# astomodynamics/cddp-cpp

Measured on AMD Instinct MI355X. Metric: trajectories_per_sec, higher is better.
Workload: dtype f64

## Files before the change

### cddp-cpp_amd/csrc/dev_models.hpp

```cpp
#pragma once
#include "dev_linalg.hpp"
#include "dev_trig.hpp"
#include "../../include/cddp_hip.h"

namespace cddp_dev {

template <int NP>
struct DualN {
  double v;
  double d[NP];
  DEV DualN() {}
  DEV DualN(double x) : v(x) {
#pragma unroll
    for (int i = 0; i < NP; ++i) d[i] = 0.0;
  }
};
template <int NP> DEV DualN<NP> operator+(const DualN<NP> &a, const DualN<NP> &b) { DualN<NP> r; r.v = a.v + b.v;
#pragma unroll
  for (int i = 0; i < NP; ++i) r.d[i] = a.d[i] + b.d[i]; return r; }
template <int NP> DEV DualN<NP> operator-(const DualN<NP> &a, const DualN<NP> &b) { DualN<NP> r; r.v = a.v - b.v;
#pragma unroll
  for (int i = 0; i < NP; ++i) r.d[i] = a.d[i] - b.d[i]; return r; }
template <int NP> DEV DualN<NP> operator-(const DualN<NP> &a) { DualN<NP> r; r.v = -a.v;
#pragma unroll
  for (int i = 0; i < NP; ++i) r.d[i] = -a.d[i]; return r; }
template <int NP> DEV DualN<NP> operator*(const DualN<NP> &a, const DualN<NP> &b) { DualN<NP> r; r.v = a.v * b.v;
#pragma unroll
  for (int i = 0; i < NP; ++i) r.d[i] = a.d[i] * b.v + a.v * b.d[i]; return r; }
template <int NP> DEV DualN<NP> operator/(const DualN<NP> &a, const DualN<NP> &b) { DualN<NP> r; r.v = a.v / b.v;
#pragma unroll
  for (int i = 0; i < NP; ++i) r.d[i] = (a.d[i] - r.v * b.d[i]) / b.v; return r; }
template <int NP> DEV DualN<NP> dsin(const DualN<NP> &a) { DualN<NP> r; double s, c; plant_sincos(a.v, &s, &c); r.v = s;
#pragma unroll
  for (int i = 0; i < NP; ++i) r.d[i] = c * a.d[i]; return r; }
template <int NP> DEV DualN<NP> dcos(const DualN<NP> &a) { DualN<NP> r; double s, c; plant_sincos(a.v, &s, &c); r.v = c; double ms = -s;
#pragma unroll
  for (int i = 0; i < NP; ++i) r.d[i] = ms * a.d[i]; return r; }
template <int NP> DEV DualN<NP> dsqrt(const DualN<NP> &a) { DualN<NP> r; r.v = sqrt(a.v); double g = 0.5 / r.v;
#pragma unroll
  for (int i = 0; i < NP; ++i) r.d[i] = g * a.d[i]; return r; }
template <int NP> DEV DualN<NP> dasin(const DualN<NP> &a) { DualN<NP> r; r.v = plant_asin(a.v); double g = 1.0 / sqrt(1.0 - a.v * a.v);
#pragma unroll
  for (int i = 0; i < NP; ++i) r.d[i] = g * a.d[i]; return r; }
template <int NP> DEV DualN<NP> dtan(const DualN<NP> &a) { DualN<NP> r; r.v = plant_tan(a.v); double g = 1.0 + r.v * r.v;
#pragma unroll
  for (int i = 0; i < NP; ++i) r.d[i] = g * a.d[i]; return r; }
DEV double dasin(double a) { return plant_asin(a); }
DEV double dtan(double a) { return plant_tan(a); }
DEV double dsin(double a) { return plant_sin(a); }
DEV double dcos(double a) { return plant_cos(a); }
DEV double dsqrt(double a) { return sqrt(a); }
DEV double dval(double a) { return a; }
template <int NP> DEV double dval(const DualN<NP> &a) { return a.v; }
DEV double lift_sin(double, double s, double) { return s; }
DEV double lift_cos(double, double, double c) { return c; }
template <int NP> DEV DualN<NP> lift_sin(const DualN<NP> &a, double s, double c) { DualN<NP> r; r.v = s;
#pragma unroll
  for (int i = 0; i < NP; ++i) r.d[i] = c * a.d[i]; return r; }
template <int NP> DEV DualN<NP> lift_cos(const DualN<NP> &a, double s, double c) { DualN<NP> r; r.v = c; const double ms = -s;
#pragma unroll
  for (int i = 0; i < NP; ++i) r.d[i] = ms * a.d[i]; return r; }
template <int N, class S> DEV void trig_n(const S *a, S *sn, S *cs) {
  double av[N], sv[N], cv[N];
#pragma unroll
  for (int i = 0; i < N; ++i) av[i] = dval(a[i]);
  sincos_n<N>(av, sv, cv);
#pragma unroll
  for (int i = 0; i < N; ++i) { sn[i] = lift_sin(a[i], sv[i], cv[i]); cs[i] = lift_cos(a[i], sv[i], cv[i]); }
}

template <int NP>
struct Dual2N {
  double v, d[NP], h[NP * NP];
  DEV Dual2N() {}
  DEV Dual2N(double x) : v(x) {
    for (int i = 0; i < NP; ++i) d[i] = 0.0;
    for (int i = 0; i < NP * NP; ++i) h[i] = 0.0;
  }
};
template <int NP> DEV Dual2N<NP> d2_unary(const Dual2N<NP> &a, double val, double p1, double p2) {
  Dual2N<NP> r; r.v = val;
  for (int i = 0; i < NP; ++i) { r.d[i] = p1 * a.d[i]; for (int j = 0; j < NP; ++j) r.h[i * NP + j] = p2 * a.d[i] * a.d[j] + p1 * a.h[i * NP + j]; }
  return r;
}
template <int NP> DEV Dual2N<NP> operator+(const Dual2N<NP> &a, const Dual2N<NP> &b) { Dual2N<NP> r; r.v = a.v + b.v;
  for (int i = 0; i < NP; ++i) r.d[i] = a.d[i] + b.d[i];
  for (int i = 0; i < NP * NP; ++i) r.h[i] = a.h[i] + b.h[i]; return r; }
template <int NP> DEV Dual2N<NP> operator-(const Dual2N<NP> &a, const Dual2N<NP> &b) { Dual2N<NP> r; r.v = a.v - b.v;
// ... 45 lines not shown
      D xs[NX], us[NU], xd[NX];
      for (int v = 0; v < NP; ++v) {
        D z(v < NX ? x[v] : u[v - NX]);
        const int blk = v / BS, off = v - blk * BS;
        if (blk == I) z.d[off] = 1.0;
        else if (blk == J) z.d[BS + off] = 1.0;
        if (v < NX) xs[v] = z; else us[v - NX] = z;
      }
      F::template eval<D>(p, xs, us, xd);
      for (int pass = 0; pass < (I == J ? 1 : 2); ++pass) {
        const int RB = pass == 0 ? I : J, CB = pass == 0 ? J : I;
        for (int ra = 0; ra < BS; ++ra) {
          const int va = RB * BS + ra;
          if (va >= NP) break;
          const int sa = (RB == I) ? ra : BS + ra;
          for (int cb = 0; cb < BS; ++cb) {
            const int vb = CB * BS + cb;
            if (vb >= NP) break;
            const int sb = (CB == I) ? cb : BS + cb;
            double *dst;
            if (va < NX && vb < NX) dst = Qxx + va * NX + vb;
            else if (va >= NX && vb >= NX) dst = Quu + (va - NX) * NU + (vb - NX);
            else if (va >= NX && vb < NX) dst = Qux + (va - NX) * NX + vb;
            else continue;
            double acc = *dst;
            for (int i = 0; i < NX; ++i) acc = acc + w[i] * (dt * (xd[i].h[sa * NS + sb] / div));
            *dst = acc;
          }
        }
      }
    }
  }
}

template <class M, class = void> struct HessBlocked { static constexpr bool value = false; };
template <class M> struct HessBlocked<M, decltype((void)sizeof(typename M::HessDyn))> { static constexpr bool value = true; };

template <class F, int NX, int NU>
DEV void ad_jacobian(const double *p, const double *x, const double *u, double *Fx, double *Fu) {
  typedef DualN<NX + NU> D;
  D xs[NX], us[NU], xd[NX];
#pragma unroll
  for (int i = 0; i < NX; ++i) { xs[i] = D(x[i]); xs[i].d[i] = 1.0; }
#pragma unroll
  for (int j = 0; j < NU; ++j) { us[j] = D(u[j]); us[j].d[NX + j] = 1.0; }
  F::template eval<D>(p, xs, us, xd);
#pragma unroll
  for (int i = 0; i < NX; ++i) {
#pragma unroll
    for (int j = 0; j < NX; ++j) Fx[i * NX + j] = xd[i].d[j];
#pragma unroll
    for (int j = 0; j < NU; ++j) Fu[i * NU + j] = xd[i].d[NX + j];
  }
}

struct PendulumModel {
  static constexpr int ID = CDDP_HIP_MODEL_PENDULUM, NX = 2, NU = 1;
  static constexpr bool kDiscrete = false;
  DEV static void f(const double *p, const double *x, const double *u, double *xd) {
    const double length = p[0], mass = p[1], damping = p[2], gravity = p[3];
    const double inertia = mass * length * length;
    xd[0] = x[1];
    xd[1] = (u[0] - damping * x[1] + mass * gravity * length * dsin(x[0])) / inertia;
  }
  DEV static void jac(const double *p, const double *x, const double *u, double *Fx, double *Fu) {
    const double length = p[0], mass = p[1], damping = p[2], gravity = p[3];
    Fx[0] = 0.0; Fx[1] = 1.0;
    Fx[2] = (gravity / length) * dcos(x[0]);
    Fx[3] = -damping / (mass * length * length);
    Fu[0] = 0.0; Fu[1] = 1.0 / (mass * length * length);
  }
  static constexpr bool kHasHess = true;
  DEV static void hess(const double *p, const double *x, const double *, double *Fxx, double *Fuu, double *Fux) {
    for (int i = 0; i < NX * NX * NX; ++i) Fxx[i] = 0.0;
    for (int i = 0; i < NX * NU * NU; ++i) Fuu[i] = 0.0;
    for (int i = 0; i < NX * NU * NX; ++i) Fux[i] = 0.0;
    Fxx[1 * NX * NX + 0] = -(p[3] / p[0]) * dsin(x[0]);
  }
};

struct CartPoleModel {
  static constexpr int ID = CDDP_HIP_MODEL_CARTPOLE, NX = 4, NU = 1;
  static constexpr bool kDiscrete = false;
  DEV static void f(const double *p, const double *x, const double *u, double *xd) {
    const double mc = p[0], mp = p[1], l = p[2], g = p[3];
    const double theta_dot = x[3], force = u[0];
    double s, c; plant_sincos(x[1], &s, &c);
    const double total_mass = mc + mp;
    const double den = mc + mp * s * s;
    xd[0] = x[2];
    xd[1] = theta_dot;
    xd[2] = (force + mp * s * (l * theta_dot * theta_dot + g * c)) / den;
    xd[3] = (-force * c - mp * l * theta_dot * theta_dot * c * s - total_mass * g * s) / (l * den);
  }
  DEV static void jac(const double *p, const double *x, const double *u, double *Fx, double *Fu) {
#ifdef CDDP_TRIG_SHARED
    {
      typedef DualN<5> D;
      D xs[4], us[1], xd[4];
#pragma unroll
      for (int i = 0; i < 4; ++i) { xs[i] = D(x[i]); xs[i].d[i] = 1.0; }
      us[0] = D(u[0]); us[0].d[4] = 1.0;
      f_ad<D>(p, xs, us, xd);
#pragma unroll
      for (int i = 0; i < 4; ++i) {
#pragma unroll
        for (int j = 0; j < 4; ++j) Fx[i * 4 + j] = xd[i].d[j];
        Fu[i] = xd[i].d[4];
      }
      return;
    }
#endif
    const double mc = p[0], mp = p[1], l = p[2], g = p[3], b = p[4];
    const double w = x[3], F = u[0];
    double s, c; plant_sincos(x[1], &s, &c);
    const double M = mc + mp;
    const double den = mc + mp * s * s;
    const double dden = 2.0 * mp * s * c;
    const double inner = l * w * w + g * c;
    const double num3 = F + mp * s * inner;
    const double dnum3 = mp * c * inner - mp * s * g * s;
    const double num4 = -F * c - mp * l * w * w * c * s - M * g * s - b * w;
    const double dnum4 = F * s - mp * l * w * w * (c * c - s * s) - M * g * c;
    const double den2 = den * den;
#pragma unroll
    for (int i = 0; i < 16; ++i) Fx[i] = 0.0;
    Fx[0 * 4 + 2] = 1.0;
    Fx[1 * 4 + 3] = 1.0;
    Fx[2 * 4 + 1] = (dnum3 * den - num3 * dden) / den2;
    Fx[2 * 4 + 3] = (mp * s * (2.0 * l * w)) / den;
    Fx[3 * 4 + 1] = (dnum4 * den - num4 * dden) / (l * den2);
    Fx[3 * 4 + 3] = (-2.0 * mp * l * w * c * s - b) / (l * den);
    Fu[0] = 0.0; Fu[1] = 0.0;
    Fu[2] = 1.0 / den;
    Fu[3] = -c / (l * den);
  }
  template <class S>
  DEV static void f_ad(const double *p, const S *x, const S *u, S *xd) {
    const double mc = p[0], mp = p[1], l = p[2], g = p[3], b = p[4];
    const S theta = x[1], x_dot = x[2], theta_dot = x[3], force = u[0];
    const S sin_theta = dsin(theta), cos_theta = dcos(theta);
    const double total_mass = mc + mp;
    const S den = S(mc) + S(mp) * sin_theta * sin_theta;
    xd[0] = x_dot;
    xd[1] = theta_dot;
    xd[2] = (force + S(mp) * sin_theta * (S(l) * theta_dot * theta_dot + S(g) * cos_theta)) / den;
    xd[3] = (-force * cos_theta - S(mp) * S(l) * theta_dot * theta_dot * cos_theta * sin_theta - S(total_mass) * S(g) * sin_theta - S(b) * theta_dot) / (S(l) * den);
  }
  static constexpr bool kHasHess = true;
  DEV static void hess(const double *p, const double *x, const double *u, double *Fxx, double *Fuu, double *Fux) {
    typedef Dual2N<5> D;
    D xs[4], us[1], xd[4];
    for (int i = 0; i < 4; ++i) { xs[i] = D(x[i]); xs[i].d[i] = 1.0; }
    us[0] = D(u[0]); us[0].d[4] = 1.0;
    f_ad<D>(p, xs, us, xd);
    for (int i = 0; i < 4; ++i) {
      for (int a = 0; a < 4; ++a) for (int b = 0; b < 4; ++b) Fxx[i * 16 + a * 4 + b] = xd[i].h[a * 5 + b];
      Fuu[i] = xd[i].h[4 * 5 + 4];
      for (int b = 0; b < 4; ++b) Fux[i * 4 + b] = xd[i].h[4 * 5 + b];
    }
  }
};

struct UnicycleModel {
  static constexpr int ID = CDDP_HIP_MODEL_UNICYCLE, NX = 3, NU = 2;
  static constexpr bool kDiscrete = false;
  DEV static void f(const double *, const double *x, const double *u, double *xd) {
    double s, c; plant_sincos(x[2], &s, &c);
    xd[0] = u[0] * c; xd[1] = u[0] * s; xd[2] = u[1];
  }
  DEV static void jac(const double *, const double *x, const double *u, double *Fx, double *Fu) {
    double s, c; plant_sincos(x[2], &s, &c);
#pragma unroll
    for (int i = 0; i < 9; ++i) Fx[i] = 0.0;
    Fx[0 * 3 + 2] = -u[0] * s;
    Fx[1 * 3 + 2] = u[0] * c;
    Fu[0] = c; Fu[1] = 0.0; Fu[2] = s; Fu[3] = 0.0; Fu[4] = 0.0; Fu[5] = 1.0;
  }
  static constexpr bool kHasHess = true;
  DEV static void hess(const double *, const double *x, const double *u, double *Fxx, double *Fuu, double *Fux) {
    double s, c; plant_sincos(x[2], &s, &c);
    for (int i = 0; i < NX * NX * NX; ++i) Fxx[i] = 0.0;
    for (int i = 0; i < NX * NU * NU; ++i) Fuu[i] = 0.0;
    for (int i = 0; i < NX * NU * NX; ++i) Fux[i] = 0.0;
    Fxx[0 * 9 + 2 * 3 + 2] = -u[0] * c;
    Fxx[1 * 9 + 2 * 3 + 2] = -u[0] * s;
    Fux[0 * 6 + 0 * 3 + 2] = -s;
    Fux[1 * 6 + 0 * 3 + 2] = c;
  }
};

template <int NX_, int NU_>
struct LTIModel {
  static constexpr int ID = CDDP_HIP_MODEL_LTI, NX = NX_, NU = NU_;
  static constexpr bool kDiscrete = true;
  static constexpr bool kHasHess = true;
  DEV static void hess(const double *, const double *, const double *, double *Fxx, double *Fuu, double *Fux) {
    for (int i = 0; i < NX * NX * NX; ++i) Fxx[i] = 0.0;
    for (int i = 0; i < NX * NU * NU; ++i) Fuu[i] = 0.0;
    for (int i = 0; i < NX * NU * NX; ++i) Fux[i] = 0.0;
  }
  DEV static void step(const double *p, const double *x, const double *u, double *xn) {
#pragma unroll
    for (int i = 0; i < NX; ++i) {
      double s = 0.0, t = 0.0;
#pragma unroll
      for (int j = 0; j < NX; ++j) s += p[i * NX + j] * x[j];
#pragma unroll
      for (int j = 0; j < NU; ++j) t += p[NX * NX + i * NU + j] * u[j];
      xn[i] = s + t;
    }
  }
  DEV static void f(const double *, const double *, const double *, double *) {}
  DEV static void jac(const double *p, const double *, const double *, double *Fx, double *Fu) {
    const double dt = p[NX * NX + NX * NU];
#pragma unroll
    for (int i = 0; i < NX; ++i)
#pragma unroll
      for (int j = 0; j < NX; ++j) Fx[i * NX + j] = (p[i * NX + j] - (i == j ? 1.0 : 0.0)) / dt;
#pragma unroll
    for (int i = 0; i < NX * NU; ++i) Fu[i] = p[NX * NX + i] / dt;
  }
};

struct BicycleDyn {
  template <class S>
  DEV static void eval(const double *p, const S *x, const S *u, S *xd) {
    const S theta = x[2], v = x[3];
    xd[0] = v * dcos(theta);
    xd[1] = v * dsin(theta);
    xd[2] = (v / S(p[0])) * dtan(u[1]);
    xd[3] = u[0];
  }
};
struct BicycleModel {
  static constexpr int ID = CDDP_HIP_MODEL_BICYCLE, NX = 4, NU = 2;
  static constexpr bool kDiscrete = false;
  static constexpr bool kHasHess = true;
  DEV static void f(const double *p, const double *x, const double *u, double *xd) { BicycleDyn::eval<double>(p, x, u, xd); }
  DEV static void jac(const double *p, const double *x, const double *u, double *Fx, double *Fu) {
    double s, c; plant_sincos(x[2], &s, &c);
    const double v = x[3], L = p[0], cd = plant_cos(u[1]);
#pragma unroll
    for (int i = 0; i < NX * NX; ++i) Fx[i] = 0.0;
#pragma unroll
    for (int i = 0; i < NX * NU; ++i) Fu[i] = 0.0;
    Fx[0 * NX + 2] = -v * s; Fx[0 * NX + 3] = c;
    Fx[1 * NX + 2] = v * c;  Fx[1 * NX + 3] = s;
    Fx[2 * NX + 3] = plant_tan(u[1]) / L;
    Fu[3 * NU + 0] = 1.0;
    Fu[2 * NU + 1] = v / (L * (cd * cd));
// ... 834 lines not shown
      for (int i = 0; i < NX; ++i) xn[i] = x[i] + dt * k1[i];
      return;
    }
    double xt[NX], k2[NX];
    if (integrator == CDDP_HIP_HEUN) {
#pragma unroll
      for (int i = 0; i < NX; ++i) xt[i] = x[i] + dt * k1[i];
      Model::f(p, xt, u, k2);
#pragma unroll
      for (int i = 0; i < NX; ++i) xn[i] = x[i] + (0.5 * dt) * (k1[i] + k2[i]);
      return;
    }
    double k3[NX];
    if (integrator == CDDP_HIP_RK3) {
#pragma unroll
      for (int i = 0; i < NX; ++i) xt[i] = x[i] + (0.5 * dt) * k1[i];
      Model::f(p, xt, u, k2);
#pragma unroll
      for (int i = 0; i < NX; ++i) xt[i] = (x[i] - dt * k1[i]) + (2 * dt) * k2[i];
      Model::f(p, xt, u, k3);
#pragma unroll
      for (int i = 0; i < NX; ++i) xn[i] = x[i] + (dt / 6) * ((k1[i] + 4.0 * k2[i]) + k3[i]);
      return;
    }
    double k4[NX];
#pragma unroll
    for (int i = 0; i < NX; ++i) xt[i] = x[i] + (0.5 * dt) * k1[i];
    Model::f(p, xt, u, k2);
#pragma unroll
    for (int i = 0; i < NX; ++i) xt[i] = x[i] + (0.5 * dt) * k2[i];
    Model::f(p, xt, u, k3);
#pragma unroll
    for (int i = 0; i < NX; ++i) xt[i] = x[i] + dt * k3[i];
    Model::f(p, xt, u, k4);
#pragma unroll
    for (int i = 0; i < NX; ++i) xn[i] = x[i] + (dt / 6) * (((k1[i] + 2.0 * k2[i]) + 2.0 * k3[i]) + k4[i]);
  }
  DEV static void step(const DynCtx &c, const double *x, const double *u, double *xn) {
    constexpr int NX = Model::NX;
    const double *p = c.mp;
    double k1[NX];
    Model::f(p, x, u, k1);
    if (c.integrator == CDDP_HIP_EULER) {
#pragma unroll
      for (int i = 0; i < NX; ++i) xn[i] = x[i] + c.dt * k1[i];
      return;
    }
    double xt[NX], k2[NX];
    if (c.integrator == CDDP_HIP_HEUN) {
#pragma unroll
      for (int i = 0; i < NX; ++i) xt[i] = x[i] + c.dt * k1[i];
      Model::f(p, xt, u, k2);
#pragma unroll
      for (int i = 0; i < NX; ++i) xn[i] = x[i] + c.hdt * (k1[i] + k2[i]);
      return;
    }
    double k3[NX];
    if (c.integrator == CDDP_HIP_RK3) {
#pragma unroll
      for (int i = 0; i < NX; ++i) xt[i] = x[i] + c.hdt * k1[i];
      Model::f(p, xt, u, k2);
#pragma unroll
      for (int i = 0; i < NX; ++i) xt[i] = (x[i] - c.dt * k1[i]) + c.dt2 * k2[i];
      Model::f(p, xt, u, k3);
#pragma unroll
      for (int i = 0; i < NX; ++i) xn[i] = x[i] + c.dt6 * ((k1[i] + 4.0 * k2[i]) + k3[i]);
      return;
    }
    double k4[NX];
#pragma unroll
    for (int i = 0; i < NX; ++i) xt[i] = x[i] + c.hdt * k1[i];
    Model::f(p, xt, u, k2);
#pragma unroll
    for (int i = 0; i < NX; ++i) xt[i] = x[i] + c.hdt * k2[i];
    Model::f(p, xt, u, k3);
#pragma unroll
    for (int i = 0; i < NX; ++i) xt[i] = x[i] + c.dt * k3[i];
    Model::f(p, xt, u, k4);
#pragma unroll
    for (int i = 0; i < NX; ++i) xn[i] = x[i] + c.dt6 * (((k1[i] + 2.0 * k2[i]) + 2.0 * k3[i]) + k4[i]);
  }
};

}
```

### cddp-cpp_amd/csrc/dev_trig.hpp

```cpp
#pragma once
#include <cmath>

#ifndef DEV
#define DEV inline
#define CDDP_TRIG_HOST 1
#endif

namespace cddp_dev {

constexpr double kTrigFastLimit = 1.0e9;

struct SinCosPair { double s, c; };

DEV SinCosPair sincos_fast(double x) {
  const double TWO_OVER_PI = 0x1.45f306dc9c883p-1;
  const double P1 = 0x1.921fb54442d18p+0, P2 = 0x1.1a62633145c07p-54, P3 = -0x1.f1976b7ed8fbcp-110;
  const double dn = __builtin_rint(x * TWO_OVER_PI);
  const double r0 = __builtin_fma(-dn, P1, x);
  const double p = dn * P2;
  const double pe = __builtin_fma(dn, P2, -p);
  const double r = r0 - p;
  const double bb = r - r0;
  const double e1 = (r0 - (r - bb)) + (-p - bb);
  const double y = __builtin_fma(-dn, P3, e1 - pe);
  const double z = r * r, w = z * z;
  const double S1 = -1.66666666666666324348e-01, S2 = 8.33333333332248946124e-03, S3 = -1.98412698298579493134e-04,
               S4 = 2.75573137070700676789e-06, S5 = -2.50507602534068634195e-08, S6 = 1.58969099521155010221e-10;
  const double rs = S2 + z * (S3 + z * S4) + z * w * (S5 + z * S6);
  const double v = z * r;
  const double ks = r - ((z * (0.5 * y - v * rs) - y) - v * S1);
  const double C1 = 4.16666666666666019037e-02, C2 = -1.38888888888741095749e-03, C3 = 2.48015872894767294178e-05,
               C4 = -2.75573143513906633035e-07, C5 = 2.08757232129817482790e-09, C6 = -1.13596475577881948265e-11;
  const double rc = z * (C1 + z * (C2 + z * C3)) + (w * w) * (C4 + z * (C5 + z * C6));
  const double hz = 0.5 * z;
  const double w1 = 1.0 - hz;
  const double kc = w1 + (((1.0 - w1) - hz) + (z * rc - r * y));
  const int n = (int)dn;
  const bool swap = (n & 1) != 0;
  double s = swap ? kc : ks, c = swap ? ks : kc;
  if (n & 2) s = -s;
  if ((n + 1) & 2) c = -c;
  SinCosPair o; o.s = s; o.c = c;
  return o;
}

#ifndef CDDP_TRIG_HOST
__device__ __attribute__((noinline)) inline void sincos_libm(double a, double *s, double *c) { sincos(a, s, c); }
#endif

template <int N>
DEV void sincos_n(const double *a, double *s, double *c) {
  bool slow = false;
#pragma unroll
  for (int i = 0; i < N; ++i) {
    const SinCosPair r = sincos_fast(a[i]);
    s[i] = r.s; c[i] = r.c;
    slow = slow || !(__builtin_fabs(a[i]) < kTrigFastLimit);
  }
#ifdef CDDP_TRIG_HOST
  if (slow)
    for (int i = 0; i < N; ++i)
      if (!(__builtin_fabs(a[i]) < kTrigFastLimit)) { s[i] = std::sin(a[i]); c[i] = std::cos(a[i]); }
#else
  if (__builtin_expect(__builtin_amdgcn_ballot_w64(slow) != 0ull, 0)) {
#pragma unroll
    for (int i = 0; i < N; ++i) {
      double ts, tc;
      sincos_libm(a[i], &ts, &tc);
      const bool out = !(__builtin_fabs(a[i]) < kTrigFastLimit);
      s[i] = out ? ts : s[i];
      c[i] = out ? tc : c[i];
    }
  }
#endif
}

DEV void sincos_1(double a, double *s, double *c) { sincos_n<1>(&a, s, c); }

DEV double bits_to_double(unsigned long long u) { double d; __builtin_memcpy(&d, &u, 8); return d; }
DEV unsigned long long double_to_bits(double d) { unsigned long long u; __builtin_memcpy(&u, &d, 8); return u; }

DEV bool log_fast_ok(double x) { return x >= 0x1p-1022 && x <= 0x1.fffffffffffffp+1023; }
DEV double log_fast_k(double x, int k0) {
  const double ln2_hi = 6.93147180369123816490e-01, ln2_lo = 1.90821492927058770002e-10;
  const double Lg1 = 6.666666666666735130e-01, Lg2 = 3.999999999940941908e-01, Lg3 = 2.857142874366239149e-01,
               Lg4 = 2.222219843214978396e-01, Lg5 = 1.818357216161805012e-01, Lg6 = 1.531383769920937332e-01,
               Lg7 = 1.479819860511658591e-01;
  unsigned long long u = double_to_bits(x);
  unsigned hx = (unsigned)(u >> 32);
  hx += 0x3ff00000u - 0x3fe6a09eu;
  const int k = (int)(hx >> 20) - 0x3ff + k0;
  hx = (hx & 0x000fffffu) + 0x3fe6a09eu;
  u = ((unsigned long long)hx << 32) | (u & 0xffffffffull);
  const double f = bits_to_double(u) - 1.0;
  const double hfsq = 0.5 * f * f;
  const double s = f / (2.0 + f);
  const double z = s * s, w = z * z;
  const double t1 = w * (Lg2 + w * (Lg4 + w * Lg6));
  const double t2 = z * (Lg1 + w * (Lg3 + w * (Lg5 + w * Lg7)));
  const double R = t2 + t1;
  const double dk = (double)k;
  return s * (hfsq + R) + dk * ln2_lo - hfsq + f + dk * ln2_hi;
}
DEV double log_fast(double x) { return log_fast_k(x, 0); }

DEV bool exp_fast_ok(double x) { return __builtin_fabs(x) <= 700.0; }
DEV double exp_fast(double x) {
  const double invln2 = 1.44269504088896338700e+00, ln2hi = 6.93147180369123816490e-01, ln2lo = 1.90821492927058770002e-10;
  const double P1 = 1.66666666666666019037e-01, P2 = -2.77777777770155933842e-03, P3 = 6.61375632143793436117e-05,
               P4 = -1.65339022054652515390e-06, P5 = 4.13813679705723846039e-08;
  const double dk = __builtin_rint(invln2 * x);
  const double hi = x - dk * ln2hi;
  const double lo = dk * ln2lo;
  const double r = hi - lo;
  const double xx = r * r;
  const double c = r - xx * (P1 + xx * (P2 + xx * (P3 + xx * (P4 + xx * P5))));
  const double y = 1.0 + (r * c / (2.0 - c) - lo + hi);
  const int k = (int)dk;
  return y * bits_to_double((unsigned long long)(0x3ff + k) << 52);
}

DEV bool asin_fast_ok(double x) { return __builtin_fabs(x) < 0.5; }
DEV double asin_fast(double x) {
  const double pS0 = 1.66666666666666657415e-01, pS1 = -3.25565818622400915405e-01, pS2 = 2.01212532134862925881e-01,
               pS3 = -4.00555345006794114027e-02, pS4 = 7.91534994289814532176e-04, pS5 = 3.47933107596021167570e-05,
               qS1 = -2.40339491173441421878e+00, qS2 = 2.02094576023350569471e+00, qS3 = -6.88283971605453293030e-01,
               qS4 = 7.70381505559019352791e-02;
  if (__builtin_fabs(x) < 0x1p-26) return x;
// ... 75 lines not shown
```

### cddp-cpp_amd/csrc/kernels_lean.hpp

```cpp
#pragma once
#include "kernels.hpp"

namespace cddp_dev {

#define GI(t, E, e) (((((size_t)(t)) * (size_t)d.NB + (size_t)(b >> 6)) * (E) + (e)) * 64 + (size_t)(b & 63))

template <class Model, class Cons>
struct CstLayout {
  static constexpr int NX = Model::NX, NU = Model::NU;
  static constexpr int CX = 0, CU = CX + NX, WQYU = CU + NU, QYUSIR = WQYU + NU * NU, IPR = QYUSIR + NU, ICOMP = IPR + 1;
  static constexpr int WQYX = ICOMP + 1, QYXSIR = WQYX + NU * NX, WXQYX = QYXSIR + NX;
  static constexpr int SIZE = Cons::HAS_X ? (WXQYX + NX * NX) : WQYX;
};

template <class Model, class Cons, bool WITH_DERIVS>
DEV void condense_eval(const ProblemDev *__restrict__ P, const double *__restrict__ xrt, const int t, const double *x, const double *u,
                       const double *y, const double *s, const double *g, const double mu, double *A, double *Bq, double *c,
                       double *ys_out = nullptr) {
  constexpr int NX = Model::NX, NU = Model::NU, M = Cons::M;
  typedef Objective<NX, NU> Obj;
  typedef CstLayout<Model, Cons> L;
  const double s_floor = dmax(mu * 1e-3, kEpsSlack);
  double Qyx[M * NX], Qyu[M * NU];
  if constexpr (WITH_DERIVS) {
// ... 521 lines not shown
#pragma unroll
    for (int j = 0; j < NX; ++j) s += vb[(size_t)(i * NX + j) * kLS] * dx[j];
    const double lam = (lop[(size_t)i * kLS] + a_pr * vxp[(size_t)i * kLS]) + s;
    finite = finite && dfinite(lam);
    lamp[(size_t)i * kLS] = lam;
  }
  if (!finite || ((d.fail_costate_mask >> only) & 1)) d.t_success[ti] = 2;
}

template <class Model>
__global__ __launch_bounds__(64) void k_costate(DevBuf d, int a0, int na, int phase_req, int force, int first_only) {
  constexpr int NX = Model::NX;
  const int b = blockIdx.x * 64 + threadIdx.x;
  const int t = blockIdx.y;
  if (b >= d.B) return;
  if (!force && d.phase[b] != phase_req) return;
  const int cur = d.cur[b];
  constexpr int NT = NX * (NX + 1) / 2;
  double xo[NX], lo[NX], vx[NX], vt[NT];
  ld<NX>(d.X + (size_t)cur * d.planeX + GI(t, NX, 0), kLS, xo);
  ld<NX>(d.Lam + (size_t)cur * d.planeX + GI(t, NX, 0), kLS, lo);
  ld<NX>(d.Vx + GI(t, NX, 0), kLS, vx);
  costate_load_triangle<NX>(d.Vxx + GI(t, NX * NX, 0), vt);
  int a_lo = a0, a_hi = a0 + na;
  if (first_only != 0) {
    const int only = first_only == 2 ? d.cand[b] : first_surviving_trial(d, a0, na, b);
    if (only < 0) return;
    a_lo = only; a_hi = only + 1;
  }
  for (int a = a_lo; a < a_hi; ++a) {
    const size_t ti = (size_t)a * d.Bp + b;
    if (!d.t_success[ti]) continue;
    const int slot = trial_slot(cur, a);
    const double a_pr = d.t_apr[ti];
    double xn[NX], lam[NX];
    ld<NX>(d.X + (size_t)slot * d.planeX + GI(t, NX, 0), kLS, xn);
    const bool finite = costate_row_eval<NX>(lo, vx, vt, xo, xn, a_pr, lam);
    if (!finite || ((d.fail_costate_mask >> a) & 1)) d.t_success[ti] = 2;
    else st<NX>(d.Lam + (size_t)slot * d.planeX + GI(t, NX, 0), kLS, lam);
  }
}

template <int NX>
DEV void costate_shadow_item(const DevBuf &d, const int b, const int t) {
  if (b >= d.B) return;
  if (d.cs_stampv[b] != d.cs_want) return;
  const int cur = d.cs_old[b], slot = d.cs_new[b];
  const double a_pr = d.cs_apr[b];
  double xo[NX], lo[NX], vx[NX], xn[NX], lam[NX], vt[NX * (NX + 1) / 2];
  ld<NX>(d.X + (size_t)cur * d.planeX + GI(t, NX, 0), kLS, xo);
  ld<NX>(d.Lam + (size_t)cur * d.planeX + GI(t, NX, 0), kLS, lo);
  ld<NX>(d.Vx_prev + GI(t, NX, 0), kLS, vx);
  costate_load_triangle<NX>(d.Vxx_prev + GI(t, NX * NX, 0), vt);
  ld<NX>(d.X + (size_t)slot * d.planeX + GI(t, NX, 0), kLS, xn);
  const bool finite = costate_row_eval<NX>(lo, vx, vt, xo, xn, a_pr, lam);
  if (!finite || (d.cs_fail_stamp != 0 && d.cs_fail_stamp == (d.cs_want | 1))) *d.cs_bad = 1;
  else st<NX>(d.Lam + (size_t)slot * d.planeX + GI(t, NX, 0), kLS, lam);
}

template <class Model>
__global__ __launch_bounds__(64) void k_costate_flush(DevBuf d) {
  costate_shadow_item<Model::NX>(d, blockIdx.x * 64 + threadIdx.x, blockIdx.y);
}

template <int NX>
__global__ __launch_bounds__(64) void k_value_merge(DevBuf d) {
  const int b = blockIdx.x * 64 + threadIdx.x, t = blockIdx.y;
  if (b >= d.B || d.cs_vbuf[b] == d.cs_vsel) return;
  double vx[NX], vxx[NX * NX];
  ld<NX>(d.Vx2 + GI(t, NX, 0), kLS, vx);
  ld<NX * NX>(d.Vxx2 + GI(t, NX * NX, 0), kLS, vxx);
  st<NX>(d.Vx + GI(t, NX, 0), kLS, vx);
  st<NX * NX>(d.Vxx + GI(t, NX * NX, 0), kLS, vxx);
}
#ifdef CDDP_K4_TIMING
__device__ unsigned long long g_k4_times[16384 * 4];
#define K4_TIME_BEGIN const unsigned long long k4_t0 = wall_clock64();
#define K4_TIME_END(role, steps) do { if (lane == 0) { const size_t k4_i = ((size_t)blockIdx.y * gridDim.x + blockIdx.x) * 4 + (role) * 2; \
    g_k4_times[k4_i] = wall_clock64() - k4_t0; g_k4_times[k4_i + 1] = (unsigned long long)(steps); } } while (0)
#else
#define K4_TIME_BEGIN
#define K4_TIME_END(role, steps)
#endif
template <class Model, class Cons, bool TERM = false, int NC = 1>
__global__ __launch_bounds__(64 * (1 + NC)) void k_forward_ipddp_pc(DevBuf d, const ProblemDev *__restrict__ Pk, const double *__restrict__ xrt,
                                                                    int a0, int phase_req, int force) {
  constexpr int NX = Model::NX, NU = Model::NU, M = Cons::M;
  typedef Objective<NX, NU> Obj;
  static_assert(M > 0, "two-role rollout is for path-constrained problems");
  constexpr int RW = 2 * NX + NU;
  constexpr int kRing = RW <= 10 ? 8 : (RW <= 20 ? 4 : 2);
  __shared__ double s_ring[kRing * RW * 64];
  static_assert(NC == 1 || NC == 2, "one or two consumer waves");
  __shared__ int s_prod;
  __shared__ int s_consv[2];
  [[maybe_unused]] __shared__ int s_abort;
  [[maybe_unused]] __shared__ int s_done1;
  constexpr int kL2 = NC > 1 ? 64 : 1;
  [[maybe_unused]] __shared__ int s_pfail[kL2], s_palive[kL2];
  [[maybe_unused]] __shared__ double s_pmax[4 * kL2];
  [[maybe_unused]] __shared__ double s_prun[kL2];
  __shared__ int s_pstat[64];
  __shared__ double s_pcost[64];
  __shared__ double s_xN[TERM ? NX * 64 : 1];
  __shared__ double s_obj[Obj::kStage];
  const int lane = threadIdx.x & 63;
  K4_TIME_BEGIN
  const int wave = __builtin_amdgcn_readfirstlane((int)threadIdx.x) >> 6;
  const bool producer = wave == 0;
  [[maybe_unused]] const int ci = NC > 1 ? wave - 1 : 0;
  int *const s_cons = &s_consv[0];
  const int b = blockIdx.x * 64 + lane;
  const int a = a0 + blockIdx.y;
  const ProblemDev *__restrict__ P = Pk;
  const cddp_hip_options &o = P->opt;
  const int N = d.N;
  const bool active = (b < d.B) && (force || d.phase[b] == phase_req);
  if (__builtin_amdgcn_ballot_w64(active) == 0ull) return;
  if (producer) { s_pstat[lane] = N + 2; if (lane == 0) { s_prod = 0; s_consv[0] = 0; s_consv[1] = 0; if constexpr (NC > 1) { s_abort = 0x7fffffff; s_done1 = 0; } } }
  Obj::stage(P, s_obj, (int)threadIdx.x, 64 * (1 + NC));
  __syncthreads();
  const int bb = (b < d.B) ? b : 0;
  const int cur = (b < d.B) ? d.cur[b] : 0;
  const int slot = trial_slot(cur, a);
  const double *Xc = d.X + (size_t)cur * d.planeX;
  const double alpha = P->alphas[a];
  const double a_pr = dmin(alpha, d.apr_max[bb]);
  auto wait_ge = [&](int *ctr, int need) -> int {
    int v;
    while ((v = __hip_atomic_load(ctr, __ATOMIC_RELAXED, __HIP_MEMORY_SCOPE_WORKGROUP)) < need) __builtin_amdgcn_s_sleep(1);
    asm volatile("" ::: "memory");
    return v;
  };
  const int kAbort = 2 * N + kRing;

  if (producer) {
    double *Xn = d.X + (size_t)slot * d.planeX;
    double *Un = d.U + (size_t)slot * d.planeU;
    const double *Uc = d.U + (size_t)cur * d.planeU;
    bool alive = active;
    double x[NX];
    ld<NX>(Xc + GI(0, NX, 0), kLS, x);
    st<NX>(Xn + GI(0, NX, 0), kLS, x);
    struct StepIn { double xo[NX], uo[NU], kk[NU], KK[NU * NX]; };
    auto load_step = [&](int tt, StepIn &r) {
      ld<NX>(Xc + GI(tt, NX, 0), kLS, r.xo);
      ld<NU>(Uc + GI(tt, NU, 0), kLS, r.uo);
      ld<NU>(d.k + GI(tt, NU, 0), kLS, r.kk);
      ld<NU * NX>(d.K + GI(tt, NU * NX, 0), kLS, r.KK);
    };
    DynCtx dc;
    dc.load(P->integrator, P->dt, P->mp);
    [[maybe_unused]] typename Obj::Ctx oc_p;
    [[maybe_unused]] double run_cost_p = 0.0;
    if constexpr (NC > 1) Obj::load_staged(P, oc_p, s_obj);
    auto prime = [&]() {
      double z[NX];
#pragma unroll
      for (int i = 0; i < NX; ++i) z[i] = 0.0;
      st<NU>(Un + GI(0, NU, 0), kLS, z);
      st<NX>(Xn + GI(1, NX, 0), kLS, z);
    };
    constexpr bool kPing = sizeof(StepIn) <= 40 * sizeof(double);
    constexpr bool kEarly = !kPing && sizeof(StepIn) <= 96 * sizeof(double);
    constexpr bool kChunkP = !kPing && !kEarly;
    struct PChunk { double K[NX], uo, kk; };
    auto load_pchunk = [&](int tt, const int i, PChunk &c) {
      ld<NX>(d.K + GI(tt, NU * NX, i * NX), kLS, c.K);
      c.uo = Uc[GI(tt, NU, i)]; c.kk = d.k[GI(tt, NU, i)];
    };
    PChunk pk0, pk1;
    double xo_c[NX];
    auto step = [&](const int t, StepIn &cs, StepIn &nxt) {
      if constexpr (kPing) {
        const int tn = t + 1 < N ? t + 1 : N - 1;
        load_step(tn, nxt);
      }
      PIPELINE_FENCE();
      double dx[NX], u[NU], xn[NX];
      bool finite = true;
      if constexpr (kChunkP) {
#pragma unroll
        for (int i = 0; i < NX; ++i) dx[i] = x[i] - xo_c[i];
#pragma unroll
        for (int i = 0; i < NU; ++i) {
          if (i + 1 < NU) { if ((i & 1) == 0) load_pchunk(t, i + 1, pk1); else load_pchunk(t, i + 1, pk0); }
          __builtin_amdgcn_sched_barrier(0);
          const PChunk &c = (i & 1) == 0 ? pk0 : pk1;
          double s1 = 0.0;
#pragma unroll
          for (int j = 0; j < NX; ++j) s1 += c.K[j] * dx[j];
          u[i] = (c.uo + a_pr * c.kk) + s1;
          finite = finite && dfinite(u[i]);
          __builtin_amdgcn_sched_barrier(0);
        }
      } else {
#pragma unroll
      for (int i = 0; i < NX; ++i) dx[i] = x[i] - cs.xo[i];
#pragma unroll
      for (int i = 0; i < NU; ++i) {
        double s1 = 0.0;
#pragma unroll
        for (int j = 0; j < NX; ++j) s1 += cs.KK[i * NX + j] * dx[j];
        u[i] = (cs.uo[i] + a_pr * cs.kk[i]) + s1;
        finite = finite && dfinite(u[i]);
      }
      }
      if (t >= kRing && (t % (kRing / 2)) == 0) {
        if (wait_ge(s_cons, t - kRing / 2) >= kAbort) alive = false;
        if constexpr (NC > 1) { if (wait_ge(&s_consv[1], t - kRing / 2) >= kAbort) alive = false; }
      }
      {
        double *rs = s_ring + (size_t)(t % kRing) * RW * 64 + lane;
#pragma unroll
        for (int i = 0; i < NX; ++i) { rs[i * 64] = x[i]; rs[(NX + i) * 64] = dx[i]; }
#pragma unroll
        for (int i = 0; i < NU; ++i) rs[(2 * NX + i) * 64] = u[i];
        if (alive && !finite) { s_pstat[lane] = t; alive = false; }
        RING_FENCE();
        __hip_atomic_store(&s_prod, t + 1, __ATOMIC_RELAXED, __HIP_MEMORY_SCOPE_WORKGROUP);
      }
      if constexpr (NC > 1) run_cost_p += Obj::running_cost(oc_p, xrt, t, x, u);
      if constexpr (kEarly) {
        load_step(t + 1 < N ? t + 1 : t, cs);
        PIPELINE_FENCE();
      }
      if constexpr (kChunkP) {
        const int tn = t + 1 < N ? t + 1 : t;
        ld<NX>(Xc + GI(tn, NX, 0), kLS, xo_c);
        load_pchunk(tn, 0, pk0);
        PIPELINE_FENCE();
      }
      Stepper<Model>::step(dc, x, u, xn);
#pragma unroll
      for (int i = 0; i < NX; ++i) finite = finite && dfinite(xn[i]);
      if (alive && !finite) { s_pstat[lane] = t; alive = false; }
      st<NU>(Un + GI(t, NU, 0), kLS, u);
      st<NX>(Xn + GI(t + 1, NX, 0), kLS, xn);
      if (alive) {
#pragma unroll
        for (int i = 0; i < NX; ++i) x[i] = xn[i];
      }
    };
    StepIn ra;
    int t = 0;
    if constexpr (kPing) {
      StepIn R[2];
#pragma unroll
      for (int j = 0; j < 1; ++j) load_step(j < N ? j : N - 1, R[j]);
      prime();
      for (; t + 1 < N; t += 2) {
#pragma unroll
        for (int j = 0; j <= 1; ++j) step(t + j, R[j], R[(j + 1) % 2]);
        if (__builtin_amdgcn_ballot_w64(alive) == 0ull) { t = N; break; }
      }
#pragma unroll
      for (int j = 0; j <= 1; ++j) if (t + j < N) step(t + j, R[j], R[(j + 1) % 2]);
    } else {
      if constexpr (kChunkP) { ld<NX>(Xc + GI(0, NX, 0), kLS, xo_c); load_pchunk(0, 0, pk0); } else load_step(0, ra);
      prime();
      for (; t < N; ++t) {
        step(t, ra, ra);
        if (__builtin_amdgcn_ballot_w64(alive) == 0ull) break;
      }
    }
    if (alive) s_pcost[lane] = Obj::terminal_cost(P, x);
    if constexpr (NC > 1) s_prun[lane] = run_cost_p;
    if constexpr (TERM) {
#pragma unroll
      for (int i = 0; i < NX; ++i) s_xN[i * 64 + lane] = x[i];
    }
    asm volatile("s_waitcnt lgkmcnt(0)" ::: "memory");
    __hip_atomic_store(&s_prod, N + kRing + 1, __ATOMIC_RELAXED, __HIP_MEMORY_SCOPE_WORKGROUP);
    K4_TIME_END(0, t);
    return;
  }

  const double *Sc = d.S + (size_t)cur * d.planeM;
  const double *Yc = d.Y + (size_t)cur * d.planeM;
  double *Sn = d.S + (size_t)slot * d.planeM;
  double *Yn = d.Y + (size_t)slot * d.planeM;
  double *Gn = d.G + (size_t)slot * d.planeM;
  const double mu = d.mu[bb];
  const double tau = dmax(o.barrier_min_fraction_to_boundary, 1.0 - mu);
  const double a_du = dmin(alpha, d.adu_max[bb]);
  const size_t ti = (size_t)a * d.Bp + bb;
  bool alive = active;
  int seen_prod = 0;
  int fail_t = N;
  if (alive && ci == 0) {
    atomicAdd(d.launched, 1ull);
    d.t_apr[ti] = a_pr; d.t_adu[ti] = a_du;
    d.t_success[ti] = 0;
    d.t_cost[ti] = d.cost[b]; d.t_merit[ti] = d.phi[b]; d.t_theta[ti] = d.theta[b];
    d.t_inf_pr[ti] = 0.0; d.t_inf_comp[ti] = 0.0;
  }
  double ev_total0 = 0.0, ev_max = 0.0, ev_icomp = 0.0, ys_lo = INFINITY, ys_hi = -INFINITY, run_cost = 0.0;
  const bool l2norm = o.ipddp_theta_norm_l2 != 0;
  struct StepIn { double xo[Cons::HAS_X ? NX : 1], uo[Cons::NEEDS_U ? NU : 1], s[M], y[M], ksv[M], ky[M], KK[NU * NX], ys[M]; };
  auto load_step = [&](int tt, StepIn &r) {
    if constexpr (Cons::HAS_X) ld<NX>(Xc + GI(tt, NX, 0), kLS, r.xo);
    if constexpr (Cons::NEEDS_U) ld<NU>(d.U + (size_t)cur * d.planeU + GI(tt, NU, 0), kLS, r.uo);
    ld<M>(Sc + GI(tt, M, 0), kLS, r.s);
    ld<M>(Yc + GI(tt, M, 0), kLS, r.y);
    ld<M>(d.ks + GI(tt, M, 0), kLS, r.ksv);
    ld<M>(d.ky + GI(tt, M, 0), kLS, r.ky);
    ld<NU * NX>(d.K + GI(tt, NU * NX, 0), kLS, r.KK);
    ld<M>(d.ys + GI(tt, M, 0), kLS, r.ys);
  };
  typename Cons::Ctx cc;
  Cons::load(P, cc);
  typename Obj::Ctx oc;
  Obj::load_staged(P, oc, s_obj);
  auto prime = [&]() {
    double z[M];
#pragma unroll
    for (int i = 0; i < M; ++i) z[i] = 0.0;
    const int tp = (NC > 1 && ci < N) ? ci : 0;
    st<M>(Sn + GI(tp, M, 0), kLS, z);
    st<M>(Yn + GI(tp, M, 0), kLS, z);
    st<M>(Gn + GI(tp, M, 0), kLS, z);
    double *ev = d.ev + GI((size_t)a * N + tp, 2 * Cons::NSEG, 0);
#pragma unroll
    for (int c = 0; c < Cons::NSEG; ++c) { if (c > 0 || NC > 1) ev[(size_t)(Cons::NSEG + c) * kLS] = 0.0; ev[(size_t)c * kLS] = 0.0; }
  };
  constexpr bool kPing = sizeof(StepIn) <= 40 * sizeof(double);
  constexpr bool kEarly = !kPing && sizeof(StepIn) <= 96 * sizeof(double);
  constexpr bool kChunk = !kPing && !kEarly && UDiag<Cons>::value && M == 2 * NU;
  struct Chunk { double K[NX], s[2], y[2], ksv[2], ky[2], ys[2]; };
  auto load_chunk = [&](int tt, const int i, Chunk &c) {
    ld<NX>(d.K + GI(tt, NU * NX, i * NX), kLS, c.K);
#pragma unroll
    for (int h = 0; h < 2; ++h) {
      const int r = i + h * NU;
      c.s[h] = Sc[GI(tt, M, r)]; c.y[h] = Yc[GI(tt, M, r)];
      c.ksv[h] = d.ks[GI(tt, M, r)]; c.ky[h] = d.ky[GI(tt, M, r)]; c.ys[h] = d.ys[GI(tt, M, r)];
    }
  };
  Chunk ck0, ck1;
  auto step = [&](const int t, StepIn &cs, StepIn &nxt) {
    if constexpr (kPing) {
      const int tn = t + NC < N ? t + NC : N - 1;
      load_step(tn, nxt);
    } else if constexpr (!kEarly && !kChunk) load_step(t, cs);
    PIPELINE_FENCE();
    if (seen_prod < t + 1) seen_prod = __builtin_amdgcn_readfirstlane(wait_ge(&s_prod, t + 1));
    double rx[NX], dx[NX], u[NU];
// ... 276 lines not shown
```

Measured before the change: 106,800.

## Specialize forward rollout on integrator and defer trig range fallback to wave-level redo

In the ping-pong forward rollout, the integrator choice is hoisted out of the time loop by dispatching to a template instantiated per integrator. Model dynamics for cartpole and unicycle gain a trig policy that uses the fast sincos and only records whether any argument was out of range. When any lane reports that, a noinline checked step recomputes the result. Load and store addresses become incrementing pointers instead of per-step index arithmetic. This aims to cut per-step branching, the inline libm fallback and address math, at the cost of more template instantiations, code size and register pressure.

```diff
diff --git a/cddp-cpp_amd/csrc/dev_models.hpp b/cddp-cpp_amd/csrc/dev_models.hpp
--- a/cddp-cpp_amd/csrc/dev_models.hpp
+++ b/cddp-cpp_amd/csrc/dev_models.hpp
@@ -1,9 +1,25 @@
 #pragma once
+#include <type_traits>
 #include "dev_linalg.hpp"
 #include "dev_trig.hpp"
 #include "../../include/cddp_hip.h"
 
 namespace cddp_dev {
+
+struct TrigChecked {
+  DEV void sincos(double a, double *s, double *c) const { plant_sincos(a, s, c); }
+};
+struct TrigFlagged {
+  bool *out_of_range;
+  DEV void sincos(double a, double *s, double *c) const { const SinCosPair r = sincos_fast_flag(a, *out_of_range); *s = r.s; *c = r.c; }
+};
+#ifdef CDDP_TRIG_SHARED
+constexpr bool kTrigFlaggable = true;
+#else
+constexpr bool kTrigFlaggable = false;
+#endif
+template <class Model, class = void> struct HasTrigPolicy { static constexpr bool value = false; };
+template <class Model> struct HasTrigPolicy<Model, typename std::enable_if<Model::kTrigPolicy>::type> { static constexpr bool value = kTrigFlaggable; };
 
 template <int NP>
 struct DualN {
@@ -215,10 +231,12 @@
 struct CartPoleModel {
   static constexpr int ID = CDDP_HIP_MODEL_CARTPOLE, NX = 4, NU = 1;
   static constexpr bool kDiscrete = false;
-  DEV static void f(const double *p, const double *x, const double *u, double *xd) {
+  static constexpr bool kTrigPolicy = true;
+  template <class Trig = TrigChecked>
+  DEV static void f(const double *p, const double *x, const double *u, double *xd, const Trig tg = Trig()) {
     const double mc = p[0], mp = p[1], l = p[2], g = p[3];
     const double theta_dot = x[3], force = u[0];
-    double s, c; plant_sincos(x[1], &s, &c);
+    double s, c; tg.sincos(x[1], &s, &c);
     const double total_mass = mc + mp;
     const double den = mc + mp * s * s;
     xd[0] = x[2];
@@ -298,8 +316,10 @@
 struct UnicycleModel {
   static constexpr int ID = CDDP_HIP_MODEL_UNICYCLE, NX = 3, NU = 2;
   static constexpr bool kDiscrete = false;
-  DEV static void f(const double *, const double *x, const double *u, double *xd) {
-    double s, c; plant_sincos(x[2], &s, &c);
+  static constexpr bool kTrigPolicy = true;
+  template <class Trig = TrigChecked>
+  DEV static void f(const double *, const double *x, const double *u, double *xd, const Trig tg = Trig()) {
+    double s, c; tg.sincos(x[2], &s, &c);
     xd[0] = u[0] * c; xd[1] = u[0] * s; xd[2] = u[1];
   }
   DEV static void jac(const double *, const double *x, const double *u, double *Fx, double *Fu) {
@@ -1300,4 +1320,56 @@
   }
 };
 
+template <class Model, bool FLAGGED, class Trig>
+DEV void roll_f(const double *p, const double *x, const double *u, double *xd, const Trig tg) {
+  if constexpr (FLAGGED) Model::f(p, x, u, xd, tg);
+  else Model::f(p, x, u, xd);
 }
+template <class Model, int INTEG, bool FLAGGED = HasTrigPolicy<Model>::value>
+DEV void roll_step(const DynCtx &c, const double *x, const double *u, double *xn, bool *redo) {
+  if constexpr (Model::kDiscrete) {
+    Stepper<Model>::step(c, x, u, xn);
+  } else {
+    constexpr int NX = Model::NX;
+    const double *p = c.mp;
+    const TrigFlagged tg{redo};
+    double k1[NX];
+    roll_f<Model, FLAGGED>(p, x, u, k1, tg);
+    if constexpr (INTEG == CDDP_HIP_EULER) {
+#pragma unroll
+      for (int i = 0; i < NX; ++i) xn[i] = x[i] + c.dt * k1[i];
+    } else if constexpr (INTEG == CDDP_HIP_HEUN) {
+      double xt[NX], k2[NX];
+#pragma unroll
+      for (int i = 0; i < NX; ++i) xt[i] = x[i] + c.dt * k1[i];
+      roll_f<Model, FLAGGED>(p, xt, u, k2, tg);
+#pragma unroll
+      for (int i = 0; i < NX; ++i) xn[i] = x[i] + c.hdt * (k1[i] + k2[i]);
+    } else if constexpr (INTEG == CDDP_HIP_RK3) {
+      double xt[NX], k2[NX], k3[NX];
+#pragma unroll
+      for (int i = 0; i < NX; ++i) xt[i] = x[i] + c.hdt * k1[i];
+      roll_f<Model, FLAGGED>(p, xt, u, k2, tg);
+#pragma unroll
+      for (int i = 0; i < NX; ++i) xt[i] = (x[i] - c.dt * k1[i]) + c.dt2 * k2[i];
+      roll_f<Model, FLAGGED>(p, xt, u, k3, tg);
+#pragma unroll
+      for (int i = 0; i < NX; ++i) xn[i] = x[i] + c.dt6 * ((k1[i] + 4.0 * k2[i]) + k3[i]);
+    } else {
+      double xt[NX], k2[NX], k3[NX], k4[NX];
+#pragma unroll
+      for (int i = 0; i < NX; ++i) xt[i] = x[i] + c.hdt * k1[i];
+      roll_f<Model, FLAGGED>(p, xt, u, k2, tg);
+#pragma unroll
+      for (int i = 0; i < NX; ++i) xt[i] = x[i] + c.hdt * k2[i];
+      roll_f<Model, FLAGGED>(p, xt, u, k3, tg);
+#pragma unroll
+      for (int i = 0; i < NX; ++i) xt[i] = x[i] + c.dt * k3[i];
+      roll_f<Model, FLAGGED>(p, xt, u, k4, tg);
+#pragma unroll
+      for (int i = 0; i < NX; ++i) xn[i] = x[i] + c.dt6 * (((k1[i] + 2.0 * k2[i]) + 2.0 * k3[i]) + k4[i]);
+    }
+  }
+}
+
+}
diff --git a/cddp-cpp_amd/csrc/dev_trig.hpp b/cddp-cpp_amd/csrc/dev_trig.hpp
--- a/cddp-cpp_amd/csrc/dev_trig.hpp
+++ b/cddp-cpp_amd/csrc/dev_trig.hpp
@@ -44,6 +44,42 @@
   return o;
 }
 
+DEV SinCosPair sincos_fast_flag(double x, bool &out_of_range) {
+  const double TWO_OVER_PI = 0x1.45f306dc9c883p-1;
+  const double P1 = 0x1.921fb54442d18p+0, P2 = 0x1.1a62633145c07p-54, P3 = -0x1.f1976b7ed8fbcp-110;
+  const double dn = __builtin_rint(x * TWO_OVER_PI);
+  const double r0 = __builtin_fma(-dn, P1, x);
+  const double p = dn * P2;
+  const double pe = __builtin_fma(dn, P2, -p);
+  const double r = r0 - p;
+  const double bb = r - r0;
+  const double e1 = (r0 - (r - bb)) + (-p - bb);
+  const double y = __builtin_fma(-dn, P3, e1 - pe);
+  const double z = r * r, w = z * z;
+  const double S1 = -1.66666666666666324348e-01, S2 = 8.33333333332248946124e-03, S3 = -1.98412698298579493134e-04,
+               S4 = 2.75573137070700676789e-06, S5 = -2.50507602534068634195e-08, S6 = 1.58969099521155010221e-10;
+  const double rs = S2 + z * (S3 + z * S4) + z * w * (S5 + z * S6);
+  const double v = z * r;
+  const double ks = r - ((z * (0.5 * y - v * rs) - y) - v * S1);
+  const double C1 = 4.16666666666666019037e-02, C2 = -1.38888888888741095749e-03, C3 = 2.48015872894767294178e-05,
+               C4 = -2.75573143513906633035e-07, C5 = 2.08757232129817482790e-09, C6 = -1.13596475577881948265e-11;
+  const double rc = z * (C1 + z * (C2 + z * C3)) + (w * w) * (C4 + z * (C5 + z * C6));
+  const double hz = 0.5 * z;
+  const double w1 = 1.0 - hz;
+  const double kc = w1 + (((1.0 - w1) - hz) + (z * rc - r * y));
+  const int n = (int)dn;
+  const bool swap = (n & 1) != 0;
+  const double s = swap ? kc : ks, c = swap ? ks : kc;
+  unsigned long long us, uc;
+  __builtin_memcpy(&us, &s, 8); __builtin_memcpy(&uc, &c, 8);
+  us ^= (unsigned long long)((unsigned)n & 2u) << 62;
+  uc ^= (unsigned long long)(((unsigned)n + 1u) & 2u) << 62;
+  SinCosPair o;
+  __builtin_memcpy(&o.s, &us, 8); __builtin_memcpy(&o.c, &uc, 8);
+  out_of_range = out_of_range || !(__builtin_fabs(x) < kTrigFastLimit);
+  return o;
+}
+
 #ifndef CDDP_TRIG_HOST
 __device__ __attribute__((noinline)) inline void sincos_libm(double a, double *s, double *c) { sincos(a, s, c); }
 #endif
diff --git a/cddp-cpp_amd/csrc/kernels_lean.hpp b/cddp-cpp_amd/csrc/kernels_lean.hpp
--- a/cddp-cpp_amd/csrc/kernels_lean.hpp
+++ b/cddp-cpp_amd/csrc/kernels_lean.hpp
@@ -627,6 +627,15 @@
 #define K4_TIME_BEGIN
 #define K4_TIME_END(role, steps)
 #endif
+template <int NX, int NU> struct RollIn { double x[NX], u[NU]; };
+template <int NX> struct RollOut { double xn[NX]; };
+template <class Model>
+__device__ __attribute__((noinline)) RollOut<Model::NX> roll_step_checked(int integrator, double dt, const double *mp, RollIn<Model::NX, Model::NU> in) {
+  RollOut<Model::NX> o;
+  Stepper<Model>::step(integrator, dt, mp, in.x, in.u, o.xn);
+  return o;
+}
+
 template <class Model, class Cons, bool TERM = false, int NC = 1>
 __global__ __launch_bounds__(64 * (1 + NC)) void k_forward_ipddp_pc(DevBuf d, const ProblemDev *__restrict__ Pk, const double *__restrict__ xrt,
                                                                     int a0, int phase_req, int force) {
@@ -688,11 +697,24 @@
     ld<NX>(Xc + GI(0, NX, 0), kLS, x);
     st<NX>(Xn + GI(0, NX, 0), kLS, x);
     struct StepIn { double xo[NX], uo[NU], kk[NU], KK[NU * NX]; };
+    const size_t rs1 = (size_t)d.NB * 64;
+    const double *ld_X = Xc + GI(0, NX, 0), *ld_U = Uc + GI(0, NU, 0), *ld_k = d.k + GI(0, NU, 0), *ld_K = d.K + GI(0, NU * NX, 0);
+    double *st_U = Un + GI(0, NU, 0), *st_X = Xn + GI(1, NX, 0);
     auto load_step = [&](int tt, StepIn &r) {
       ld<NX>(Xc + GI(tt, NX, 0), kLS, r.xo);
       ld<NU>(Uc + GI(tt, NU, 0), kLS, r.uo);
       ld<NU>(d.k + GI(tt, NU, 0), kLS, r.kk);
       ld<NU * NX>(d.K + GI(tt, NU * NX, 0), kLS, r.KK);
+    };
+    auto load_row = [&](StepIn &r) {
+      ld<NX>(ld_X, kLS, r.xo);
+      ld<NU>(ld_U, kLS, r.uo);
+      ld<NU>(ld_k, kLS, r.kk);
+      ld<NU * NX>(ld_K, kLS, r.KK);
+    };
+    auto advance_ld = [&](const int t) {
+      const size_t s = t + 1 < N ? rs1 : 0;
+      ld_X += s * NX; ld_U += s * NU; ld_k += s * NU; ld_K += s * (NU * NX);
     };
     DynCtx dc;
     dc.load(P->integrator, P->dt, P->mp);
@@ -716,10 +738,12 @@
     };
     PChunk pk0, pk1;
     double xo_c[NX];
-    auto step = [&](const int t, StepIn &cs, StepIn &nxt) {
+    constexpr bool kFlagged = kPing && HasTrigPolicy<Model>::value && NC == 1;
+    auto step = [&](auto integ, const int t, StepIn &cs, StepIn &nxt) {
+      constexpr int INTEG = decltype(integ)::value;
       if constexpr (kPing) {
-        const int tn = t + 1 < N ? t + 1 : N - 1;
-        load_step(tn, nxt);
+        advance_ld(t);
+        load_row(nxt);
       }
       PIPELINE_FENCE();
       double dx[NX], u[NU], xn[NX];
@@ -776,38 +800,66 @@
         load_pchunk(tn, 0, pk0);
         PIPELINE_FENCE();
       }
-      Stepper<Model>::step(dc, x, u, xn);
+      [[maybe_unused]] bool redo = false;
+      if constexpr (kPing) roll_step<Model, INTEG, kFlagged>(dc, x, u, xn, &redo);
+      else Stepper<Model>::step(dc, x, u, xn);
+      if constexpr (kFlagged) {
+        if (__builtin_expect(__builtin_amdgcn_ballot_w64(redo) != 0ull, 0)) {
+          RollIn<NX, NU> in;
+#pragma unroll
+          for (int i = 0; i < NX; ++i) in.x[i] = x[i];
+#pragma unroll
+          for (int i = 0; i < NU; ++i) in.u[i] = u[i];
+          const RollOut<NX> o = roll_step_checked<Model>(dc.integrator, dc.dt, P->mp, in);
+#pragma unroll
+          for (int i = 0; i < NX; ++i) xn[i] = o.xn[i];
+        }
+      }
 #pragma unroll
       for (int i = 0; i < NX; ++i) finite = finite && dfinite(xn[i]);
       if (alive && !finite) { s_pstat[lane] = t; alive = false; }
-      st<NU>(Un + GI(t, NU, 0), kLS, u);
-      st<NX>(Xn + GI(t + 1, NX, 0), kLS, xn);
+      if constexpr (kPing) {
+        st<NU>(st_U, kLS, u);
+        st<NX>(st_X, kLS, xn);
+        st_U += rs1 * NU; st_X += rs1 * NX;
+      } else {
+        st<NU>(Un + GI(t, NU, 0), kLS, u);
+        st<NX>(Xn + GI(t + 1, NX, 0), kLS, xn);
+      }
       if (alive) {
 #pragma unroll
         for (int i = 0; i < NX; ++i) x[i] = xn[i];
       }
     };
-    StepIn ra;
     int t = 0;
-    if constexpr (kPing) {
-      StepIn R[2];
-#pragma unroll
-      for (int j = 0; j < 1; ++j) load_step(j < N ? j : N - 1, R[j]);
-      prime();
-      for (; t + 1 < N; t += 2) {
-#pragma unroll
-        for (int j = 0; j <= 1; ++j) step(t + j, R[j], R[(j + 1) % 2]);
-        if (__builtin_amdgcn_ballot_w64(alive) == 0ull) { t = N; break; }
-      }
-#pragma unroll
-      for (int j = 0; j <= 1; ++j) if (t + j < N) step(t + j, R[j], R[(j + 1) % 2]);
-    } else {
-      if constexpr (kChunkP) { ld<NX>(Xc + GI(0, NX, 0), kLS, xo_c); load_pchunk(0, 0, pk0); } else load_step(0, ra);
-      prime();
-      for (; t < N; ++t) {
-        step(t, ra, ra);
-        if (__builtin_amdgcn_ballot_w64(alive) == 0ull) break;
-      }
+    auto walk = [&](auto integ) {
+      if constexpr (kPing) {
+        StepIn R[2];
+        load_row(R[0]);
+        prime();
+        for (; t + 1 < N; t += 2) {
+#pragma unroll
+          for (int j = 0; j <= 1; ++j) step(integ, t + j, R[j], R[(j + 1) % 2]);
+          if (__builtin_amdgcn_ballot_w64(alive) == 0ull) { t = N; break; }
+        }
+#pragma unroll
+        for (int j = 0; j <= 1; ++j) if (t + j < N) step(integ, t + j, R[j], R[(j + 1) % 2]);
+      } else {
+        StepIn ra;
+        if constexpr (kChunkP) { ld<NX>(Xc + GI(0, NX, 0), kLS, xo_c); load_pchunk(0, 0, pk0); } else load_step(0, ra);
+        prime();
+        for (; t < N; ++t) {
+          step(integ, t, ra, ra);
+          if (__builtin_amdgcn_ballot_w64(alive) == 0ull) break;
+        }
+      }
+    };
+    if constexpr (Model::kDiscrete || !kPing) walk(std::integral_constant<int, CDDP_HIP_RK4>());
+    else switch (dc.integrator) {
+      case CDDP_HIP_EULER: walk(std::integral_constant<int, CDDP_HIP_EULER>()); break;
+      case CDDP_HIP_HEUN: walk(std::integral_constant<int, CDDP_HIP_HEUN>()); break;
+      case CDDP_HIP_RK3: walk(std::integral_constant<int, CDDP_HIP_RK3>()); break;
+      default: walk(std::integral_constant<int, CDDP_HIP_RK4>()); break;
     }
     if (alive) s_pcost[lane] = Obj::terminal_cost(P, x);
     if constexpr (NC > 1) s_prun[lane] = run_cost_p;
```

Result: faster. 110,800, median of 6 (+3.7%).
